# siesta-tool/SequenceDetectionQueryExecutor

Hardware: NVIDIA B200
Metric: events scanned/sec (/detection verification) (higher is better)
Workload: dtype int32

## Files before the change

### include/siesta_gpu.h

```cpp
#ifndef SIESTA_GPU_H
#define SIESTA_GPU_H

#include <stdint.h>

#ifdef __cplusplus
extern "C" {
#endif

#define SIESTA_OK 0
#define SIESTA_E_INVALID (-1)
#define SIESTA_E_CUDA (-2)
#define SIESTA_E_UNSUPPORTED (-3)
#define SIESTA_E_NOMEM (-4)
#define SIESTA_E_REFERENCE_THROWS (-5)

const char* siesta_last_error(void);

#define SIESTA_STATE_NORMAL 0
#define SIESTA_STATE_KLEENE_PLUS 1
#define SIESTA_STATE_KLEENE_STAR 2
#define SIESTA_STATE_NEGATIVE 3
#define SIESTA_STATE_OR 4

#define SIESTA_ATTR_POSITION 0
// ... 73 lines not shown
int siesta_init(int32_t device_id, siesta_ctx** out);
void siesta_shutdown(siesta_ctx* ctx);

int siesta_log_load(siesta_ctx* ctx, const int64_t* trace_off, const int32_t* act,
                    const int64_t* ts_ms, int64_t n_traces, int64_t n_events,
                    int32_t n_activities, siesta_log** out);
int siesta_log_wrap_device(siesta_ctx* ctx, const int64_t* d_trace_off, const int32_t* d_act,
                           const int64_t* d_ts_ms, int64_t n_traces, int64_t n_events,
                           int32_t n_activities, int32_t max_trace_len, siesta_log** out);
void siesta_log_set_first_trace(siesta_log* log, int64_t first_trace);
#define SIESTA_MAX_BLOCKS 16
int siesta_log_set_blocks(siesta_log* log, int32_t n_blocks, const int64_t* local_first, const int64_t* global_first);
void siesta_log_free(siesta_log* log);
int64_t siesta_log_n_traces(const siesta_log* log);
int64_t siesta_log_n_events(const siesta_log* log);

int siesta_log_filter_time(siesta_log* log, int64_t from_ms, int32_t has_from, int64_t till_ms, int32_t has_till,
                           siesta_log** out);
int siesta_log_group(siesta_log* log, const int64_t* group_off, const int64_t* group_traces, int32_t n_groups,
                     const int32_t* types, int32_t n_types, siesta_log** out, int32_t* group_ids, int32_t* n_kept);
int siesta_log_source_events(siesta_log* log, int64_t* out);

int siesta_log_append(siesta_log* log, const int64_t* trace_idx, const int64_t* batch_off, int64_t n_listed,
                      const int32_t* act, const int64_t* ts_ms, int64_t n_new_traces, int32_t n_activities,
                      siesta_log** out, double* kernel_ms);
int siesta_log_read(siesta_log* log, int64_t t0, int64_t t1, int64_t* trace_off, int32_t* act, int64_t* ts_ms);

#define SIESTA_F_RETURN_ALL 1u
#define SIESTA_F_ONLY_APPEARANCES 2u
#define SIESTA_F_MODE_HEAD 4u
// ... 199 lines not shown
```

### sequencedetectionqueryexecutor_b200/_lib.py

```python
import ctypes as C
import os

from . import _abi

_HERE = os.path.dirname(os.path.abspath(__file__))
LIB_PATH = os.environ.get("SIESTA_GPU_LIB") or os.path.join(_HERE, "libsiesta_gpu.so")
_lib = None

EXPORTS = [
    "siesta_last_error", "siesta_pattern_compile", "siesta_init", "siesta_shutdown", "siesta_log_load",
    "siesta_log_wrap_device", "siesta_log_free", "siesta_log_n_traces", "siesta_log_n_events", "siesta_detect",
    "siesta_matches_free", "siesta_evaluate_events", "siesta_evaluate_events_act8", "siesta_detect_device", "siesta_detect_device_begin", "siesta_detect_device_finish", "siesta_dev_matches_free",
    "siesta_kernel_launches", "siesta_declare_counts_size", "siesta_declare_counts", "siesta_declare_counts_device",
    "siesta_index_load", "siesta_index_build", "siesta_index_free", "siesta_index_list_len", "siesta_index_get_list",
    "siesta_intersect", "siesta_intersect_device", "siesta_device_free", "siesta_pattern_extract_pairs",
    "siesta_candidates", "siesta_candidates_device", "siesta_pair_stats", "siesta_pair_stats_device",
    "siesta_explore_accurate", "siesta_why_not_match", "siesta_almost_matches_free", "siesta_log_set_first_trace", "siesta_log_set_blocks",
    "siesta_packed_block_bytes", "siesta_dev_matches_pack",
    "siesta_exchange_create", "siesta_exchange_export", "siesta_exchange_import", "siesta_exchange_connect_local",
    "siesta_exchange_free", "siesta_exchange_required_bytes", "siesta_detect_allgather", "siesta_exchange_allreduce_i64",
    "siesta_multi_init", "siesta_multi_shutdown", "siesta_multi_n_devices", "siesta_multi_log_load", "siesta_multi_log_free",
    "siesta_multi_log_shard", "siesta_multi_detect", "siesta_multi_declare_counts", "siesta_multi_why_not_match",
    "siesta_log_filter_time", "siesta_log_group", "siesta_log_source_events",
    "siesta_log_append", "siesta_log_read", "siesta_multi_log_append",
]


class SiestaError(RuntimeError):
    def __init__(self, code, msg):
        super().__init__(f"libsiesta_gpu error {code}: {msg}")
        self.code = code


def lib():
    global _lib
    if _lib is not None:
        return _lib
    if not os.path.exists(LIB_PATH):
        raise ImportError(f"{LIB_PATH} is missing: build it with `make -C {os.path.join(_HERE, 'csrc')}` "
# ... 8 lines not shown
    L.siesta_shutdown.restype = None
    L.siesta_log_load.argtypes = [vp, vp, vp, vp, i64, i64, i32, P(vp)]
    L.siesta_log_wrap_device.argtypes = [vp, vp, vp, vp, i64, i64, i32, i32, P(vp)]
    L.siesta_packed_block_bytes.argtypes = [i64, i64, i64, i64, i32]
    L.siesta_packed_block_bytes.restype = i64
    L.siesta_dev_matches_pack.argtypes = [vp, P(_abi.DevMatches), u32, i64, vp, i64, vp]
    L.siesta_log_set_first_trace.argtypes = [vp, i64]
    L.siesta_log_set_first_trace.restype = None
    L.siesta_log_set_blocks.argtypes = [vp, i32, P(i64), P(i64)]
    L.siesta_log_free.argtypes = [vp]
    L.siesta_log_free.restype = None
    L.siesta_log_n_traces.argtypes = [vp]
    L.siesta_log_n_traces.restype = i64
    L.siesta_log_n_events.argtypes = [vp]
    L.siesta_log_n_events.restype = i64
    L.siesta_detect.argtypes = [vp, P(_abi.Nfa), vp, i64, u32, P(P(_abi.Matches))]
    L.siesta_matches_free.argtypes = [P(_abi.Matches)]
    L.siesta_matches_free.restype = None
    L.siesta_evaluate_events.argtypes = [vp, vp, vp, vp, i64, i64, i32, P(_abi.Nfa), u32, P(P(_abi.Matches))]
    L.siesta_evaluate_events_act8.argtypes = [vp, vp, vp, vp, i64, i64, i32, P(_abi.Nfa), u32, P(P(_abi.Matches))]
    L.siesta_detect_device.argtypes = [vp, P(_abi.Nfa), vp, i64, u32, vp, P(_abi.DevMatches)]
    L.siesta_detect_device_begin.argtypes = [vp, P(_abi.Nfa), vp, i64, u32, vp, P(vp)]
    L.siesta_detect_device_finish.argtypes = [vp, P(_abi.DevMatches)]
    L.siesta_dev_matches_free.argtypes = [P(_abi.DevMatches)]
    L.siesta_dev_matches_free.restype = None
    L.siesta_kernel_launches.restype = i64
    L.siesta_declare_counts_size.argtypes = [i32, i32]
    L.siesta_declare_counts_size.restype = i64
    L.siesta_declare_counts.argtypes = [vp, i32, vp, P(C.c_double)]
    L.siesta_declare_counts_device.argtypes = [vp, i32, vp, vp, P(C.c_double)]
# ... 58 lines not shown
```

### sequencedetectionqueryexecutor_b200/api.py

```python
import ctypes as C

import numpy as np

from . import _abi
from ._lib import check, lib


def _ptr(a):
    return C.c_void_p(a.ctypes.data) if a is not None else None


def _batch(trace_idx, batch_off, act, ts_ms):
    out = (np.ascontiguousarray(trace_idx, dtype=np.int64), np.ascontiguousarray(batch_off, dtype=np.int64),
           np.ascontiguousarray(act, dtype=np.int32), np.ascontiguousarray(ts_ms, dtype=np.int64))
    if len(out[1]) != len(out[0]) + 1:
        raise ValueError("batch_off must have one entry more than trace_idx")
    if len(out[2]) != len(out[3]):
        raise ValueError("act and ts_ms must have the same length")
    if out[1][-1] != len(out[2]):
        raise ValueError(f"batch_off[-1] = {int(out[1][-1])} but act / ts_ms hold {len(out[2])} events")
    return out


class Context:
# ... 60 lines not shown
            self._keep = device_tensors
            check(lib().siesta_log_wrap_device(ctx._h, C.c_void_p(d_off.data_ptr()), C.c_void_p(d_act.data_ptr()),
                                               C.c_void_p(d_ts.data_ptr()), d_off.numel() - 1, d_act.numel(),
                                               self.n_activities, int(max_trace_len), C.byref(self._h)))
        self.n_traces = lib().siesta_log_n_traces(self._h)
        self.n_events = lib().siesta_log_n_events(self._h)

    @classmethod
    def _adopt(cls, ctx, handle, n_activities):
        self = cls.__new__(cls)
        self.ctx, self._h, self.n_activities, self._keep = ctx, handle, int(n_activities), None
        self.n_traces = lib().siesta_log_n_traces(handle)
        self.n_events = lib().siesta_log_n_events(handle)
        return self

    def filter_time(self, from_ms=None, till_ms=None):
        h = C.c_void_p()
        check(lib().siesta_log_filter_time(self._h, int(from_ms or 0), 0 if from_ms is None else 1, int(till_ms or 0),
                                           0 if till_ms is None else 1, C.byref(h)))
        return EventLog._adopt(self.ctx, h, self.n_activities)

    def group(self, groups, types):
        off = np.zeros(len(groups) + 1, dtype=np.int64)
        np.cumsum([len(g) for g in groups], out=off[1:])
        flat = np.array([t for g in groups for t in g], dtype=np.int64)
        ty = np.asarray(sorted(set(types)), dtype=np.int32)
        gids = np.zeros(max(len(groups), 1), dtype=np.int32)
        h, k = C.c_void_p(), C.c_int32(0)
        check(lib().siesta_log_group(self._h, _ptr(off), _ptr(flat) if len(flat) else None, len(groups), _ptr(ty), len(ty), C.byref(h),
                                     _ptr(gids), C.byref(k)))
# ... 382 lines not shown
```

### sequencedetectionqueryexecutor_b200/csrc/append.cu

```cuda
#include <algorithm>
#include <cstring>
#include <string>
#include <vector>

#include "common.cuh"

namespace siesta {

constexpr int AP_T = 256;
constexpr int64_t AP_TILE = 8192;

__global__ void __launch_bounds__(AP_T) ap_offsets_kernel(const int64_t* __restrict__ old_off, int64_t T, int64_t T2,
                                                         const int64_t* __restrict__ tidx, const int64_t* __restrict__ boff,
                                                         int64_t k, int64_t* __restrict__ new_off, int64_t* __restrict__ P,
                                                         unsigned long long* max_len) {
    const int64_t t = (int64_t)blockIdx.x * AP_T + threadIdx.x;
    unsigned long long len = 0;
    if (t <= T2) {
        int64_t lo = 0, hi = k;
        while (lo < hi) {
            const int64_t mid = (lo + hi) >> 1;
            if (tidx[mid] < t) lo = mid + 1; else hi = mid;
        }
        const int64_t o = old_off[t < T ? t : T];
// ... 191 lines not shown
    unsigned long long h_max = 0;
    if ((e = cudaGetLastError()) == cudaSuccess) e = cudaEventRecord(ev1, stream);
    if (e == cudaSuccess) e = cudaMemcpyAsync(&h_max, d_max, 8, cudaMemcpyDeviceToHost, stream);
    if (e == cudaSuccess) e = cudaStreamSynchronize(stream);
    float ms = 0.f;
    if (e == cudaSuccess) e = cudaEventElapsedTime(&ms, ev0, ev1);
    if (e != cudaSuccess) return fail(SIESTA_E_CUDA, std::string("rebuild: ") + cudaGetErrorString(e));

    Log batch;
    batch.ctx = c;
    batch.d_act = d_bact;
    batch.n_activities = n_activities;
    batch.act_valid = true;
    if (validate_act_range(&batch, 0, NB, stream) != SIESTA_OK) return fail(SIESTA_E_CUDA, siesta_last_error());
    cudaFreeAsync(stage, stream);
    cudaEventDestroy(ev0);
    cudaEventDestroy(ev1);

    Log* L = new Log();
    L->ctx = c;
    L->d_trace_off = d_off;
    L->d_act = d_act;
    L->d_ts_ms = d_ts;
    L->n_traces = T2;
    L->n_events = E2;
    L->n_activities = n_activities;
    L->max_trace_len = (int32_t)(h_max > 0x7fffffffull ? 0x7fffffffull : h_max);
    L->true_max_len = (int64_t)h_max;
    L->owns = true;
    L->first_trace = S->first_trace;
    L->act_valid = S->act_valid && batch.act_valid;
    if (kernel_ms) *kernel_ms = ms;
    *out = reinterpret_cast<siesta_log*>(L);
    return SIESTA_OK;
}

extern "C" int siesta_log_read(siesta_log* log, int64_t t0, int64_t t1, int64_t* trace_off, int32_t* act, int64_t* ts_ms) {
    Log* L = reinterpret_cast<Log*>(log);
    if (!L || !trace_off || (!act) != (!ts_ms)) {
        set_error("siesta_log_read: null argument (act and ts_ms are both given or both NULL)");
        return SIESTA_E_INVALID;
    }
    if (t0 < 0 || t1 < t0 || t1 > L->n_traces) {
        set_error("siesta_log_read: need 0 <= t0 <= t1 <= n_traces");
        return SIESTA_E_INVALID;
    }
// ... 13 lines not shown
```

### sequencedetectionqueryexecutor_b200/csrc/capi.cu

```cuda
#include <algorithm>
#include <cstdlib>
#include <cstring>
#include <vector>

#include "common.cuh"

namespace siesta {

static thread_local std::string t_last_error;
std::atomic<long long> g_kernel_launches{0};

void set_error(const std::string& msg) { t_last_error = msg; }

}

using namespace siesta;

extern "C" const char* siesta_last_error(void) { return t_last_error.c_str(); }
extern "C" int64_t siesta_kernel_launches(void) { return (int64_t)g_kernel_launches.load(); }

extern "C" int siesta_init(int32_t device_id, siesta_ctx** out) {
    if (!out) return SIESTA_E_INVALID;
    int n_dev = 0;
    cudaError_t e = cudaGetDeviceCount(&n_dev);
// ... 85 lines not shown
}
}

extern "C" void siesta_shutdown(siesta_ctx* ctx) {
    if (!ctx) return;
    Ctx* c = reinterpret_cast<Ctx*>(ctx);
    cudaSetDevice(c->device);
    cudaDeviceSynchronize();
    for (DevBlock& b : c->dev_arena) cudaFree(b.p);
    if (c->stream) cudaStreamDestroy(c->stream);
    for (HostBlock& b : c->arena) cudaFreeHost(b.p);
    for (void* p : c->pinned_slabs) cudaFreeHost(p);
    delete c;
}

__global__ void act_range_kernel(const int32_t* act, int64_t n, int32_t n_act, int* bad) {
    int any = 0;
    for (int64_t i = (int64_t)blockIdx.x * blockDim.x + threadIdx.x; i < n; i += (int64_t)gridDim.x * blockDim.x)
        any |= (unsigned)act[i] >= (unsigned)n_act;
    if (__any_sync(0xffffffffu, any) && (threadIdx.x & 31) == 0) atomicOr(bad, 1);
}

namespace siesta {
int validate_act_range(Log* L, int64_t first_event, int64_t n_events, cudaStream_t stream) {
    if (n_events == 0) return SIESTA_OK;
    Ctx* c = L->ctx;
    int* d_bad = nullptr;
    SIESTA_CUDA_OK(cudaMallocAsync((void**)&d_bad, sizeof(int), stream));
    SIESTA_CUDA_OK(cudaMemsetAsync(d_bad, 0, sizeof(int), stream));
    const int64_t want = (n_events + 255) / 256;
    const int grid = (int)(want < (int64_t)c->sm_count * 16 ? want : (int64_t)c->sm_count * 16);
    act_range_kernel<<<grid, 256, 0, stream>>>(L->d_act + first_event, n_events, L->n_activities, d_bad);
    SIESTA_LAUNCHED();
    int bad = 1;
    SIESTA_CUDA_OK(cudaMemcpyAsync(&bad, d_bad, sizeof(int), cudaMemcpyDeviceToHost, stream));
    SIESTA_CUDA_OK(cudaStreamSynchronize(stream));
    cudaFreeAsync(d_bad, stream);
    if (bad) L->act_valid = false;
    return SIESTA_OK;
}
}

__global__ void csr_check_kernel(const int64_t* off, int64_t n_traces, int64_t n_events, int* bad) {
    int any = 0;
    for (int64_t i = (int64_t)blockIdx.x * blockDim.x + threadIdx.x; i <= n_traces; i += (int64_t)gridDim.x * blockDim.x) {
        const int64_t v = off[i];
        if (v < 0 || v > n_events) any = 1;
        if (i == 0 && v != 0) any = 1;
        if (i == n_traces && v != n_events) any = 1;
        if (i < n_traces && off[i + 1] < v) any = 1;
    }
    if (__any_sync(0xffffffffu, any) && (threadIdx.x & 31) == 0) atomicOr(bad, 1);
}

// ... 7 lines not shown
        ~Free() { cudaFreeAsync(p, s); }
    } guard{d_bad, c->stream};
    SIESTA_CUDA_OK(cudaMemsetAsync(d_bad, 0, sizeof(int), c->stream));
    const int64_t want = (L->n_traces + 1 + 255) / 256;
    const int grid = (int)(want < (int64_t)c->sm_count * 16 ? want : (int64_t)c->sm_count * 16);
    csr_check_kernel<<<grid, 256, 0, c->stream>>>(L->d_trace_off, L->n_traces, L->n_events, d_bad);
    SIESTA_LAUNCHED();
    int bad = 1;
    SIESTA_CUDA_OK(cudaMemcpyAsync(&bad, d_bad, sizeof(int), cudaMemcpyDeviceToHost, c->stream));
    SIESTA_CUDA_OK(cudaStreamSynchronize(c->stream));
    if (bad) {
        set_error("siesta_log_wrap_device: trace_off must start at 0, be non-decreasing and end at n_events");
        return SIESTA_E_INVALID;
    }
    return SIESTA_OK;
}

static int validate_act(Log* L) {
    L->act_valid = true;
    return validate_act_range(L, 0, L->n_events, L->ctx->stream);
}

static int check_csr(const int64_t* trace_off, int64_t n_traces, int64_t n_events, int32_t* max_len) {
    if (n_traces < 0 || n_events < 0 || trace_off[0] != 0 || trace_off[n_traces] != n_events) {
        set_error("CSR log: trace_off must start at 0 and end at n_events");
        return SIESTA_E_INVALID;
    }
    int64_t mx = 0;
    for (int64_t t = 0; t < n_traces; ++t) {
        const int64_t len = trace_off[t + 1] - trace_off[t];
        if (len < 0) {
            set_error("CSR log: trace_off must be non-decreasing");
            return SIESTA_E_INVALID;
        }
        mx = len > mx ? len : mx;
// ... 32 lines not shown
        delete L;
        return SIESTA_E_NOMEM;
    }
    L->d_trace_off = (const int64_t*)d_off;
    L->d_act = (const int32_t*)d_act;
    L->d_ts_ms = (const int64_t*)d_ts;
    e = cudaMemcpyAsync(d_off, trace_off, (size_t)(n_traces + 1) * 8, cudaMemcpyHostToDevice, c->stream);
    if (e == cudaSuccess && n_events) e = cudaMemcpyAsync(d_act, act, (size_t)n_events * 4, cudaMemcpyHostToDevice, c->stream);
    if (e == cudaSuccess && n_events) e = cudaMemcpyAsync(d_ts, ts_ms, (size_t)n_events * 8, cudaMemcpyHostToDevice, c->stream);
    if (e == cudaSuccess) e = cudaStreamSynchronize(c->stream);
    if (e != cudaSuccess) {
        set_error(std::string("siesta_log_load: host -> device copy: ") + cudaGetErrorString(e));
        siesta_log_free(reinterpret_cast<siesta_log*>(L));
        return SIESTA_E_CUDA;
    }
    if ((rc = validate_act(L))) {
        siesta_log_free(reinterpret_cast<siesta_log*>(L));
        return rc;
    }
    *out = reinterpret_cast<siesta_log*>(L);
    return SIESTA_OK;
}

extern "C" int siesta_log_wrap_device(siesta_ctx* ctx, const int64_t* d_trace_off, const int32_t* d_act,
                                      const int64_t* d_ts_ms, int64_t n_traces, int64_t n_events, int32_t n_activities,
                                      int32_t max_trace_len, siesta_log** out) {
    if (!ctx || !d_trace_off || !out || n_traces < 0 || n_events < 0 || n_activities < 0 || (n_events > 0 && (!d_act || !d_ts_ms))) {
        set_error("siesta_log_wrap_device: bad argument (null column with n_events > 0?)");
        return SIESTA_E_INVALID;
    }
    Log* L = new Log();
    L->ctx = reinterpret_cast<Ctx*>(ctx);
    L->d_trace_off = d_trace_off;
    L->d_act = d_act;
    L->d_ts_ms = d_ts_ms;
    L->n_traces = n_traces;
    L->n_events = n_events;
    L->n_activities = n_activities;
    L->max_trace_len = max_trace_len;
    L->owns = false;
    int rc = cudaSetDevice(L->ctx->device) == cudaSuccess ? SIESTA_OK : SIESTA_E_CUDA;
    if (rc == SIESTA_OK) rc = validate_device_csr(L);
    if (rc == SIESTA_OK) rc = validate_act(L);
    if (rc) {
        delete L;
        return rc;
    }
    *out = reinterpret_cast<siesta_log*>(L);
    return SIESTA_OK;
}

extern "C" void siesta_log_set_first_trace(siesta_log* log, int64_t first_trace) {
    if (log) reinterpret_cast<Log*>(log)->first_trace = first_trace;
}

extern "C" int siesta_log_set_blocks(siesta_log* log, int32_t n_blocks, const int64_t* local_first, const int64_t* global_first) {
    Log* L = reinterpret_cast<Log*>(log);
    if (!L || n_blocks < 0 || n_blocks > SIESTA_MAX_BLOCKS || (n_blocks > 0 && (!local_first || !global_first))) {
// ... 12 lines not shown
    }
    L->n_blocks = n_blocks;
    return SIESTA_OK;
}

extern "C" void siesta_log_free(siesta_log* log) {
    if (!log) return;
    Log* L = reinterpret_cast<Log*>(log);
    if (L->owns) {
        cudaSetDevice(L->ctx->device);
        cudaFree((void*)L->d_trace_off);
        cudaFree((void*)L->d_act);
        cudaFree((void*)L->d_ts_ms);
        if (L->d_src_event) cudaFree((void*)L->d_src_event);
    }
    delete L;
}

extern "C" int64_t siesta_log_n_traces(const siesta_log* log) { return log ? reinterpret_cast<const Log*>(log)->n_traces : 0; }
extern "C" int64_t siesta_log_n_events(const siesta_log* log) { return log ? reinterpret_cast<const Log*>(log)->n_events : 0; }

namespace {
constexpr uint64_t RESULT_MAGIC = 0x5349455354414d31ull;
constexpr size_t PIN_THRESHOLD = 256 * 1024;
constexpr size_t ARENA_KEEP_BYTES = (size_t)4 << 30;

struct ResultHeader {
    uint64_t magic;
    Ctx* ctx;
    void* base;
    uint64_t pad[5];
};
static_assert(sizeof(ResultHeader) == 64, "ResultHeader is one cache line");

void* arena_alloc(Ctx* c, size_t bytes) {
// ... 332 lines not shown
            if (!ts_mapped) ok(cudaMemcpyAsync(d_ts + e0, ts_ms + e0, (size_t)(e1 - e0) * 8, cudaMemcpyHostToDevice, s_copy));
        }
        ok(cudaEventCreateWithFlags(&copied[k], cudaEventDisableTiming));
        ok(cudaEventRecord(copied[k], s_copy));
        ok(cudaStreamWaitEvent(s_prep, copied[k], 0));
        if (e1 > e0 && e == cudaSuccess) {
            const int64_t n = e1 - e0;
            if (act8) {
                const int64_t want = (n / 4 + 256) / 256;
                const int grid = (int)std::max<int64_t>(1, std::min<int64_t>(want, (int64_t)c->sm_count * 8));
                widen_act8_kernel<<<grid, 256, 0, s_prep>>>(d_act8, d_act, e0, e1);
                SIESTA_LAUNCHED();
            }
            const int64_t want = (n + 255) / 256;
            const int grid = (int)std::max<int64_t>(1, std::min<int64_t>(want, (int64_t)c->sm_count * 16));
            act_range_kernel<<<grid, 256, 0, s_prep>>>(d_act + e0, n, n_activities, d_bad + k);
            SIESTA_LAUNCHED();
        }
        ok(cudaMemcpyAsync(h_bad + k, d_bad + k, sizeof(int), cudaMemcpyDeviceToHost, s_prep));
        ok(cudaEventCreateWithFlags(&ready[k], cudaEventDisableTiming));
        ok(cudaEventRecord(ready[k], s_prep));
    };
    struct Streamed {
        bool on = false;
        char* base = nullptr;
        siesta_matches* m = nullptr;
        cudaStream_t s = nullptr;
        std::vector<cudaEvent_t> done;
        int64_t a_tr = 0, a_occ = 0, a_ev = 0, a_err = 0, a_unsup = 0, n_emit = 0;
        bool counted = true;
        double k_ms = 0, d_ms = 0;
// ... 189 lines not shown
```

### sequencedetectionqueryexecutor_b200/csrc/common.cuh

```cuda
#pragma once
#include <cuda_runtime.h>
#include <stdint.h>

#include <atomic>
#include <mutex>
#include <string>
#include <vector>

#include "../../include/siesta_gpu.h"

namespace siesta {

void set_error(const std::string& msg);
struct Ctx;
void* dev_arena_alloc(Ctx* c, size_t bytes);
void dev_arena_free(Ctx* c, void* p);
struct DevMatchesImpl {
    void* block = nullptr;
    Ctx* owner = nullptr;
};
extern std::atomic<long long> g_kernel_launches;

#define SIESTA_CUDA_OK(expr)                                                                      \
    do {                                                                                          \
// ... 33 lines not shown
    Ctx* ctx = nullptr;
    const int64_t* d_trace_off = nullptr;
    const int32_t* d_act = nullptr;
    const int64_t* d_ts_ms = nullptr;
    const int64_t* d_src_event = nullptr;
    int64_t n_traces = 0, n_events = 0;
    int32_t n_activities = 0;
    int32_t max_trace_len = 0;
    int64_t true_max_len = -1;
    bool owns = false;
    int64_t first_trace = 0;
    int32_t n_blocks = 0;
    int64_t blk_local[SIESTA_MAX_BLOCKS + 1] = {0};
    int64_t blk_global[SIESTA_MAX_BLOCKS] = {0};
    bool act_valid = false;
};

struct DevNfa {
    int32_t n_states;
    uint32_t init_st;
    uint32_t all2;
    uint8_t kind[SIESTA_MAX_STATES];
    uint8_t n_preds[SIESTA_MAX_STATES];
    uint8_t has_vv;
    uint8_t need_vv;
    uint8_t any_kleene;
    uint8_t merge_safe;
    uint8_t cross_safe;
    uint8_t fast_class;
    int8_t kmax[SIESTA_MAX_STATES + 1];
// ... 13 lines not shown
    uint8_t le[SIESTA_MAX_STATES][SIESTA_MAX_PREDS];
    uint8_t sh[SIESTA_MAX_STATES][SIESTA_MAX_PREDS];
    uint8_t cc[SIESTA_MAX_STATES][SIESTA_MAX_PREDS];
    uint8_t markov;
    uint8_t prev[SIESTA_MAX_STATES], m_ge[SIESTA_MAX_STATES], m_le[SIESTA_MAX_STATES];
};

int nkw_build(const DevNfa& dn, uint32_t flags, NkwProgram* out);

struct DetectPending;
struct RebaseOffsets {
    int64_t trace, occ, ev;
};
int detect_device_impl(Log* log, const siesta_nfa* nfa, const int64_t* d_cand, int64_t n_cand, uint32_t flags, cudaStream_t stream,
                       RebaseOffsets base, siesta_dev_matches* out);
int validate_act_range(Log* L, int64_t first_event, int64_t n_events, cudaStream_t stream);
bool append_check_batch(const char* fn, int64_t T, const int64_t* trace_idx, const int64_t* batch_off, int64_t n_listed,
                        const int32_t* act, const int64_t* ts_ms, int64_t n_new_traces);
int assemble_matches(Ctx* c, std::vector<siesta_dev_matches>& parts, uint32_t flags, cudaStream_t stream, siesta_matches** out,
                     const std::vector<Ctx*>* part_ctx);
int detect_device_finish_impl(DetectPending* q, siesta_dev_matches* out);
void detect_pending_set_base(DetectPending* q, RebaseOffsets base);

int validate_nfa(const siesta_nfa* nfa, uint32_t flags, DevNfa* out);

constexpr int XCHG_MAX_RANKS = 16;
constexpr size_t XCHG_CTRL_BYTES = 8192;
constexpr int64_t XCHG_ERR_CAP = 4096;
enum { XST_LIMITS = 1, XST_STAGING = 2, XST_RANGE = 4, XST_ERRCAP = 8, XST_TIMEOUT = 16 };
struct XHeader {
    unsigned long long seq;
// ... 32 lines not shown
```

### sequencedetectionqueryexecutor_b200/csrc/detect.cu

```cuda
#include <algorithm>
#include <cstdio>
#include <type_traits>
#include <cstdlib>
#include <cstring>
#include <vector>

#include "detect_common.cuh"

namespace siesta {

template <int W, int R, int NF, bool SMEM_RUNS>
struct WarpSmem {
    static constexpr int NE = ROWS_OF(W);
    static constexpr size_t famvv_off = 0;
    static constexpr size_t famvv_bytes = SMEM_RUNS ? sizeof(unsigned long long) * NF * 32 : 0;
    static constexpr size_t rmask_off = famvv_off + famvv_bytes;
    static constexpr size_t rmask_bytes = SMEM_RUNS ? sizeof(typename MaskOps<W>::T) * R * 32 : 0;
    typedef typename std::conditional<W == 1, uint16_t, uint32_t>::type small_t;
    static constexpr size_t small_off = rmask_off + rmask_bytes;
    static constexpr size_t small_bytes = sizeof(small_t) * NE * 32;
    static constexpr size_t rmeta_off = (small_off + small_bytes + 15) & ~(size_t)15;
    static constexpr size_t rmeta_bytes = SMEM_RUNS ? sizeof(uint32_t) * R * 32 : 0;
    static constexpr size_t bytes_off = rmeta_off + rmeta_bytes;
    static constexpr size_t bytes_bytes = SMEM_RUNS ? (size_t)(R + 3 * NF) * 32 : 0;
// ... 912 lines not shown
    DevBuf work(log->ctx);
    const size_t nn = (size_t)std::max<int64_t>(n, 1);
    size_t w_off = 0;
    auto carve = [&w_off](size_t bytes) {
        const size_t at = w_off;
        w_off += (bytes + 255) & ~(size_t)255;
        return at;
    };
    NkwProgram prog;
    const int nkw_space = nkw_build(dn, flags, &prog);
    std::vector<uint16_t> sigs;
    for (size_t a = 0; a < lut.size(); ++a) {
        const uint16_t sg = lut[a] & 0xFFu;
        if (sg && std::find(sigs.begin(), sigs.end(), sg) == sigs.end()) sigs.push_back(sg);
    }
    const bool use_nkp = nkw_space != NKW_NONE && (!needs_ts || return_all) && log->act_valid && log->n_activities <= 255 && !sigs.empty() && sigs.size() <= 7 &&
                         (reinterpret_cast<uintptr_t>(log->d_act) & 31u) == 0 && std::getenv("SIESTA_K1_NO_NKP") == nullptr;
    const size_t reg2 = use_nkp ? (size_t)std::max<int64_t>(cap_ev, n * (int64_t)std::max(1, n_positive)) : 0;
    const bool use_long = dn.fast_class == FAST_NK && std::getenv("SIESTA_K1_NO_LONG") == nullptr;
    const int64_t cap_long = use_long ? std::min<int64_t>(log->n_events, (int64_t)1 << 21) : 0;
    const size_t long_pool = use_long ? (size_t)std::min<int64_t>(std::max<int64_t>(log->n_events * 64, (int64_t)1 << 20), (int64_t)256 << 20) : 0;
    const size_t n_blk = (nn + GT - 1) / GT;
    const size_t o_ovf2 = use_nkp ? carve(nn * 8) : 0;
    const size_t o_unsup = carve((size_t)SIESTA_MAX_UNSUPPORTED * 8);
    const size_t o_unsup2 = use_long ? carve((size_t)SIESTA_MAX_UNSUPPORTED * 8) : 0;
    const size_t o_pool = carve(long_pool);
    const size_t o_nlut = use_nkp ? carve((size_t)(log->n_activities + 1) * 16) : 0;
    const size_t o_lut = carve(lut.size() * sizeof(uint16_t)), o_nocc = carve(nn * 4), o_stage = carve(nn * 8),
                 o_stage_occ = carve(return_all ? nn * 8 : 0), o_counters = carve(32 * 8), o_err = carve(nn * 8), o_ovf = carve(nn * 8),
                 o_blk = carve(n_blk * 3 * 8), o_top = carve(((n_blk + 1023) / 1024) * 3 * 8), o_occ_nev = carve(return_all ? ((size_t)(cap_occ + cap_long) + (use_nkp ? nn : 0)) * 4 : 0), o_pos = carve(((size_t)cap_ev + reg2 + (size_t)cap_long) * 4);
    size_t o_rank = 0, o_act = 0, o_ts = 0;
    if (all_cols) {
// ... 81 lines not shown
    P.ovf_list = b_ovf.as<int64_t>();
    P.blk_sums = b_blk.as<unsigned long long>();
    P.n_blk = (int64_t)n_blk;

    P.ovf_slot = 4;
    P.tile_slot = 16;
    h_cnt = pinned_counters_get(log->ctx);
    if (!h_cnt) {
        set_error("cudaHostAlloc (counters) failed");
        return SIESTA_E_NOMEM;
    }
    std::memset(h_cnt, 0, 128);
    if (n > 0) {
        if (use_nkp) {
            DetectParams N = P;
            N.ovf_list = reinterpret_cast<int64_t*>(wb + o_ovf2);
            N.ovf_slot = 13;
            N.tile_slot = 18;
            N.fix_ev = cap_ev;
            N.fix_np = std::max(1, n_positive);
            N.fix_occ = return_all ? cap_occ + cap_long : -1;
            std::vector<uint32_t> nlut((size_t)(log->n_activities + 1) * 4, 0u);
            std::memset(N.cls_word, 0, sizeof(N.cls_word));
            for (int a = 0; a <= log->n_activities; ++a) {
                const uint16_t sg = a < log->n_activities ? (lut[a] & 0xFFu) : 0;
                int c = 0;
                if (sg) {
                    c = (int)(std::find(sigs.begin(), sigs.end(), sg) - sigs.begin()) + 1;
                    N.cls_word[c] = sg;
                }
// ... 639 lines not shown
```

### sequencedetectionqueryexecutor_b200/csrc/detect_common.cuh

```cuda
#pragma once
#include "detect_fast.cuh"

namespace siesta {

constexpr int NT = 128;
constexpr int NT_MAX = 128;
#define ROWS_OF(W) ((W) == 1 ? 24 : 64)

struct DetectParams {
    const int64_t* trace_off;
    const int32_t* act;
    const int64_t* ts_ms;
    const int64_t* cand;
    const int64_t* work;
    int64_t n_work;
    const unsigned long long* n_work_dev;
    int32_t ovf_slot;
    int32_t tile_slot;
    const uint16_t* lut;
    uint32_t relrev[3][2];
    uint16_t cls_word[8];
    int32_t cls_act[8];
    int32_t n_planes;
    int64_t n_events;
// ... 5 lines not shown
    uint32_t* d_cnt;
    int64_t* d_stage;
    int64_t* d_stage_occ;
    int32_t* s_occ_nev;
    int32_t* s_ev_pos;
    int32_t* s_ev_rank;
    int32_t* s_ev_act;
    int64_t* s_ev_ts;
    int64_t cap_occ, cap_ev;
    int64_t fix_ev;
    int32_t fix_np;
    int64_t fix_occ;
    uint32_t st_inv[SIESTA_MAX_STATES][3];
    uint8_t st_single[SIESTA_MAX_STATES];
    const uint4* nkp_lut;
    int32_t tile_batch;
    unsigned long long* counters;
    unsigned long long* blk_sums;
    int64_t n_blk;
    int64_t* err_list;
    int64_t* ovf_list;
    int64_t ovf_cap;
};

__device__ __forceinline__ long long shfl_i64(long long v, int src) {
    int lo = __shfl_sync(0xffffffffu, (int)(v & 0xffffffffll), src);
    int hi = __shfl_sync(0xffffffffu, (int)(v >> 32), src);
    return ((long long)hi << 32) | (unsigned int)lo;
}

// ... 37 lines not shown
    const int none = P.n_act;
#pragma unroll
    for (int q = 0; q < 2; ++q) {
        const long long c = e + 8 * q;
        if (c >= o1) {
            v[2 * q] = v[2 * q + 1] = make_int4(none, none, none, none);
        } else {
            asm volatile("ld.global.nc.v8.s32 {%0,%1,%2,%3,%4,%5,%6,%7}, [%8];"
                         : "=r"(v[2 * q].x), "=r"(v[2 * q].y), "=r"(v[2 * q].z), "=r"(v[2 * q].w), "=r"(v[2 * q + 1].x),
                           "=r"(v[2 * q + 1].y), "=r"(v[2 * q + 1].z), "=r"(v[2 * q + 1].w)
                         : "l"(P.act + c));
        }
    }
}

__device__ __forceinline__ uint32_t rel_push32(uint32_t pend, uint32_t relrev, int a) {
    uint32_t t;
    asm("shl.b32 %0, %1, %2;" : "=r"(t) : "r"(relrev), "r"(a));
    return __funnelshift_r(t, pend, 31);
}
__device__ __forceinline__ uint32_t rel_push64(uint32_t pend, uint32_t relrev_a, uint32_t relrev_b, int a) {
    uint32_t t;
    const uint32_t w = ((unsigned)a < 32u) ? relrev_a : (((unsigned)a < 64u) ? relrev_b : 0u);
    asm("shl.b32 %0, %1, %2;" : "=r"(t) : "r"(w), "r"(a & 31));
    return __funnelshift_r(t, pend, 31);
}

template <int NPL, bool WIDE>
__device__ __forceinline__ void scan_block(const DetectParams& P, const int4 (&v)[8], uint32_t (&pl)[3]) {
#pragma unroll
// ... 31 lines not shown
```

### sequencedetectionqueryexecutor_b200/csrc/detect_nkp.cu

```cuda
#include "detect_common.cuh"

namespace siesta {

#ifndef SIESTA_NKP_MIN_CTAS
#define SIESTA_NKP_MIN_CTAS 8
#endif
#ifndef SIESTA_NKP_PREFETCH
#define SIESTA_NKP_PREFETCH 0
#endif

constexpr int LUT_SKEW = 8;
template <int NPL, bool RAW>
__device__ __forceinline__ void scan16(const uint4* __restrict__ lut, const int4 (&v)[4], uint32_t (&pl)[3], uint32_t& racc) {
#pragma unroll
    for (int q = 3; q >= 0; --q) {
        const int a[4] = {v[q].x, v[q].y, v[q].z, v[q].w};
#pragma unroll
        for (int i = 3; i >= 0; --i) {
            const uint4 w = lut[a[i] * LUT_SKEW];
            pl[0] = pl[0] * w.x + w.y;
            if (NPL > 1) pl[1] = pl[1] * w.x + w.z;
            if (NPL > 2) pl[2] = pl[2] * w.x + w.w;
            if (!RAW) racc = racc * 2u + w.x;
        }
    }
}

__device__ __forceinline__ int select32(uint32_t x, int r) {
    int pos = 0;
#pragma unroll
    for (int w = 16; w >= 1; w >>= 1) {
        const int c = __popc((x >> pos) & ((1u << w) - 1u));
        if (r >= c) {
            r -= c;
            pos += w;
        }
    }
    return pos;
}
__device__ __forceinline__ int select64(unsigned long long x, int r) {
    const uint32_t lo = (uint32_t)x, hi = (uint32_t)(x >> 32);
    const int c = __popc(lo);
    return r >= c ? 32 + select32(hi, r - c) : select32(lo, r);
}

template <int NPL, bool RAW, bool MARKOV>
__global__ void __launch_bounds__(NT_MAX, SIESTA_NKP_MIN_CTAS) detect_nkp_kernel(const __grid_constant__ DetectParams P, const __grid_constant__ NkwProgram prog) {
    typedef typename std::conditional<RAW, unsigned long long, uint32_t>::type mask_t;
    typedef unsigned long long u64;
    typedef NkwBits<mask_t> B;
    const int lane = threadIdx.x & 31;
    extern __shared__ uint4 s_lut_all[];
    for (int i = threadIdx.x; i < (P.n_act + 1) * LUT_SKEW; i += blockDim.x) s_lut_all[i] = P.nkp_lut[i / LUT_SKEW];
    __syncthreads();
    const uint4* s_lut = s_lut_all + (lane & (LUT_SKEW - 1));
    const bool evt_pos = (P.flags & SIESTA_F_EVT_POS) != 0;
    const bool all_cols = (P.flags & SIESTA_F_NO_EVENT_COLUMNS) == 0;
    const bool return_all = (P.flags & SIESTA_F_RETURN_ALL) != 0;
    const bool first_only = (P.flags & (SIESTA_F_COUNT_MATCHES | SIESTA_F_RETURN_ALL)) == 0;

    const long long n_work = P.n_work_dev ? (long long)__ldg(P.n_work_dev) : (long long)P.n_work;
    const long long n_tiles = (n_work + 31) / 32;
    const int batch = P.tile_batch;
    long long tile = 0, next_batch = 0, next_batch2 = 0;
    if (lane == 0) {
        tile = (long long)atomicAdd(P.counters + P.tile_slot, (unsigned long long)batch);
        next_batch = (long long)atomicAdd(P.counters + P.tile_slot, (unsigned long long)batch);
    }
    tile = shfl_i64(tile, 0);
    int left = batch;
// ... 20 lines not shown
        int64_t nci;
        long long no0, no1;
        locate(nxt, nci, no0, no1);
#endif

        const long long e0 = o0 & ~7LL;
        const int lead = (int)(o0 - e0);
        const long long span = (o1 - o0) + lead;
        bool fits = span <= 64 && ((o1 + 7) & ~7LL) <= P.n_events;
        const long long o1s = fits ? o1 : e0;
        u64 valid = 0;
        if (fits && o1 > o0) valid = (span == 64 ? ~0ull : ((1ull << (int)span) - 1ull)) & ~((1ull << lead) - 1ull);
        const bool second = __any_sync(0xffffffffu, fits && span > 32);

        uint32_t q[3] = {0u, 0u, 0u}, qb[3] = {0u, 0u, 0u}, ra = 0u, rb = 0u;
        {
            int4 A[4], B[4];
            if (second) {
                load_quarter(P, e0 + 48, o1s, A);
                load_quarter(P, e0 + 32, o1s, B);
                scan16<NPL, RAW>(s_lut, A, RAW ? qb : q, rb);
                load_quarter(P, e0 + 16, o1s, A);
                scan16<NPL, RAW>(s_lut, B, RAW ? qb : q, rb);
                load_quarter(P, e0, o1s, B);
                rb += 1u;
            } else {
                load_quarter(P, e0 + 16, o1s, A);
                load_quarter(P, e0, o1s, B);
            }
            scan16<NPL, RAW>(s_lut, A, q, ra);
            scan16<NPL, RAW>(s_lut, B, q, ra);
// ... 150 lines not shown
#endif
    }
    if (lane == 31) {
        if (acc_occ) {
            atomicAdd(P.counters + 0, acc_occ);
            atomicAdd(P.counters + 6, acc_occ);
        }
        if (acc_ev) atomicAdd(P.counters + 1, acc_ev);
        if (acc_emit) atomicAdd(P.counters + 2, acc_emit);
    }
}

namespace {
template <int NPL, bool RAW, bool MARKOV>
int launch_one(const Ctx* ctx, cudaStream_t stream, DetectParams P, const NkwProgram& prog) {
    auto kern = detect_nkp_kernel<NPL, RAW, MARKOV>;
    const size_t smem = (size_t)(P.n_act + 1) * LUT_SKEW * sizeof(uint4);
    int per_sm = 0;
    SIESTA_CUDA_OK(cudaOccupancyMaxActiveBlocksPerMultiprocessor(&per_sm, kern, NT, smem));
    if (per_sm < 1) per_sm = 1;
    if (const char* env = std::getenv("SIESTA_K1_CTAS_PER_SM")) {
        const int v = std::atoi(env);
        if (v >= 1 && v < per_sm) per_sm = v;
    }
    if (const char* env = std::getenv("SIESTA_NKP_CARVEOUT")) {
        const int v = std::atoi(env);
        if (v >= 0 && v <= 100) SIESTA_CUDA_OK(cudaFuncSetAttribute(kern, cudaFuncAttributePreferredSharedMemoryCarveout, v));
    }
    const int64_t n_tiles = (P.n_work + 31) / 32;
    const int64_t ctas_needed = (n_tiles + NT / 32 - 1) / (NT / 32);
    int grid = (int)std::min<int64_t>(ctas_needed, (int64_t)ctx->sm_count * per_sm);
// ... 28 lines not shown
```

Baseline: 550.6 billion.

## Add byte-packed activity column and scan it in the NKP detection kernel

Builds a uint8 copy of the activity column during log validation when there are at most 255 activities, and the NKP detection kernel reads 8-byte chunks of it instead of int32 quads. The LUT offset is taken straight from the byte with shifts and masks. This cuts the global memory traffic of the scan to a quarter, since the kernel is bandwidth bound on activity reads. In exchange it needs extra device memory and a conversion pass at load or append time, and the old path stays reachable through an environment variable.

```diff
diff --git a/include/siesta_gpu.h b/include/siesta_gpu.h
--- a/include/siesta_gpu.h
+++ b/include/siesta_gpu.h
@@ -111,6 +111,7 @@
 void siesta_log_free(siesta_log* log);
 int64_t siesta_log_n_traces(const siesta_log* log);
 int64_t siesta_log_n_events(const siesta_log* log);
+int64_t siesta_log_act8_bytes(const siesta_log* log);
 
 int siesta_log_filter_time(siesta_log* log, int64_t from_ms, int32_t has_from, int64_t till_ms, int32_t has_till,
                            siesta_log** out);
diff --git a/sequencedetectionqueryexecutor_b200/_lib.py b/sequencedetectionqueryexecutor_b200/_lib.py
--- a/sequencedetectionqueryexecutor_b200/_lib.py
+++ b/sequencedetectionqueryexecutor_b200/_lib.py
@@ -22,7 +22,7 @@
     "siesta_multi_init", "siesta_multi_shutdown", "siesta_multi_n_devices", "siesta_multi_log_load", "siesta_multi_log_free",
     "siesta_multi_log_shard", "siesta_multi_detect", "siesta_multi_declare_counts", "siesta_multi_why_not_match",
     "siesta_log_filter_time", "siesta_log_group", "siesta_log_source_events",
-    "siesta_log_append", "siesta_log_read", "siesta_multi_log_append",
+    "siesta_log_append", "siesta_log_read", "siesta_multi_log_append", "siesta_log_act8_bytes",
 ]
 
 
@@ -61,6 +61,8 @@
     L.siesta_log_n_traces.restype = i64
     L.siesta_log_n_events.argtypes = [vp]
     L.siesta_log_n_events.restype = i64
+    L.siesta_log_act8_bytes.argtypes = [vp]
+    L.siesta_log_act8_bytes.restype = i64
     L.siesta_detect.argtypes = [vp, P(_abi.Nfa), vp, i64, u32, P(P(_abi.Matches))]
     L.siesta_matches_free.argtypes = [P(_abi.Matches)]
     L.siesta_matches_free.restype = None
diff --git a/sequencedetectionqueryexecutor_b200/api.py b/sequencedetectionqueryexecutor_b200/api.py
--- a/sequencedetectionqueryexecutor_b200/api.py
+++ b/sequencedetectionqueryexecutor_b200/api.py
@@ -98,6 +98,10 @@
         self.n_events = lib().siesta_log_n_events(handle)
         return self
 
+    @property
+    def act8_bytes(self):
+        return lib().siesta_log_act8_bytes(self._h)
+
     def filter_time(self, from_ms=None, till_ms=None):
         h = C.c_void_p()
         check(lib().siesta_log_filter_time(self._h, int(from_ms or 0), 0 if from_ms is None else 1, int(till_ms or 0),
diff --git a/sequencedetectionqueryexecutor_b200/csrc/append.cu b/sequencedetectionqueryexecutor_b200/csrc/append.cu
--- a/sequencedetectionqueryexecutor_b200/csrc/append.cu
+++ b/sequencedetectionqueryexecutor_b200/csrc/append.cu
@@ -229,8 +229,7 @@
     batch.act_valid = true;
     if (validate_act_range(&batch, 0, NB, stream) != SIESTA_OK) return fail(SIESTA_E_CUDA, siesta_last_error());
     cudaFreeAsync(stage, stream);
-    cudaEventDestroy(ev0);
-    cudaEventDestroy(ev1);
+    stage = nullptr;
 
     Log* L = new Log();
     L->ctx = c;
@@ -245,6 +244,22 @@
     L->owns = true;
     L->first_trace = S->first_trace;
     L->act_valid = S->act_valid && batch.act_valid;
+    if (L->act_valid) {
+        float ms8 = 0.f;
+        e = cudaEventRecord(ev0, stream);
+        const int rc8 = e == cudaSuccess ? validate_log_act(L, stream) : SIESTA_E_CUDA;
+        if (rc8 == SIESTA_OK && (e = cudaEventRecord(ev1, stream)) == cudaSuccess && (e = cudaEventSynchronize(ev1)) == cudaSuccess)
+            e = cudaEventElapsedTime(&ms8, ev0, ev1);
+        if (rc8 != SIESTA_OK || e != cudaSuccess) {
+            const std::string why = rc8 != SIESTA_OK ? std::string(siesta_last_error()) : std::string(cudaGetErrorString(e));
+            L->owns = false;
+            siesta_log_free(reinterpret_cast<siesta_log*>(L));
+            return fail(SIESTA_E_CUDA, "byte activity column: " + why);
+        }
+        ms += ms8;
+    }
+    cudaEventDestroy(ev0);
+    cudaEventDestroy(ev1);
     if (kernel_ms) *kernel_ms = ms;
     *out = reinterpret_cast<siesta_log*>(L);
     return SIESTA_OK;
diff --git a/sequencedetectionqueryexecutor_b200/csrc/capi.cu b/sequencedetectionqueryexecutor_b200/csrc/capi.cu
--- a/sequencedetectionqueryexecutor_b200/csrc/capi.cu
+++ b/sequencedetectionqueryexecutor_b200/csrc/capi.cu
@@ -123,15 +123,18 @@
     delete c;
 }
 
-__global__ void act_range_kernel(const int32_t* act, int64_t n, int32_t n_act, int* bad) {
+__global__ void act_range_kernel(const int32_t* act, int64_t n, int32_t n_act, int* bad, uint8_t* act8) {
     int any = 0;
-    for (int64_t i = (int64_t)blockIdx.x * blockDim.x + threadIdx.x; i < n; i += (int64_t)gridDim.x * blockDim.x)
-        any |= (unsigned)act[i] >= (unsigned)n_act;
+    for (int64_t i = (int64_t)blockIdx.x * blockDim.x + threadIdx.x; i < n; i += (int64_t)gridDim.x * blockDim.x) {
+        const int32_t a = act[i];
+        any |= (unsigned)a >= (unsigned)n_act;
+        if (act8) act8[i] = (uint8_t)a;
+    }
     if (__any_sync(0xffffffffu, any) && (threadIdx.x & 31) == 0) atomicOr(bad, 1);
 }
 
 namespace siesta {
-int validate_act_range(Log* L, int64_t first_event, int64_t n_events, cudaStream_t stream) {
+int validate_act_range(Log* L, int64_t first_event, int64_t n_events, cudaStream_t stream, uint8_t* act8) {
     if (n_events == 0) return SIESTA_OK;
     Ctx* c = L->ctx;
     int* d_bad = nullptr;
@@ -139,7 +142,7 @@
     SIESTA_CUDA_OK(cudaMemsetAsync(d_bad, 0, sizeof(int), stream));
     const int64_t want = (n_events + 255) / 256;
     const int grid = (int)(want < (int64_t)c->sm_count * 16 ? want : (int64_t)c->sm_count * 16);
-    act_range_kernel<<<grid, 256, 0, stream>>>(L->d_act + first_event, n_events, L->n_activities, d_bad);
+    act_range_kernel<<<grid, 256, 0, stream>>>(L->d_act + first_event, n_events, L->n_activities, d_bad, act8);
     SIESTA_LAUNCHED();
     int bad = 1;
     SIESTA_CUDA_OK(cudaMemcpyAsync(&bad, d_bad, sizeof(int), cudaMemcpyDeviceToHost, stream));
@@ -147,6 +150,22 @@
     cudaFreeAsync(d_bad, stream);
     if (bad) L->act_valid = false;
     return SIESTA_OK;
+}
+
+int validate_log_act(Log* L, cudaStream_t stream) {
+    L->act_valid = true;
+    uint8_t* a8 = nullptr;
+    if (L->n_activities <= 255 && L->n_events > 0 && cudaMalloc((void**)&a8, (size_t)L->n_events + 64) != cudaSuccess) {
+        cudaGetLastError();
+        a8 = nullptr;
+    }
+    const int rc = validate_act_range(L, 0, L->n_events, stream, a8);
+    if (rc || !L->act_valid) {
+        cudaFree(a8);
+        a8 = nullptr;
+    }
+    L->d_act8 = a8;
+    return rc;
 }
 }
 
@@ -184,11 +203,6 @@
         return SIESTA_E_INVALID;
     }
     return SIESTA_OK;
-}
-
-static int validate_act(Log* L) {
-    L->act_valid = true;
-    return validate_act_range(L, 0, L->n_events, L->ctx->stream);
 }
 
 static int check_csr(const int64_t* trace_off, int64_t n_traces, int64_t n_events, int32_t* max_len) {
@@ -251,7 +265,7 @@
         siesta_log_free(reinterpret_cast<siesta_log*>(L));
         return SIESTA_E_CUDA;
     }
-    if ((rc = validate_act(L))) {
+    if ((rc = validate_log_act(L, c->stream))) {
         siesta_log_free(reinterpret_cast<siesta_log*>(L));
         return rc;
     }
@@ -278,7 +292,7 @@
     L->owns = false;
     int rc = cudaSetDevice(L->ctx->device) == cudaSuccess ? SIESTA_OK : SIESTA_E_CUDA;
     if (rc == SIESTA_OK) rc = validate_device_csr(L);
-    if (rc == SIESTA_OK) rc = validate_act(L);
+    if (rc == SIESTA_OK) rc = validate_log_act(L, L->ctx->stream);
     if (rc) {
         delete L;
         return rc;
@@ -321,11 +335,19 @@
         cudaFree((void*)L->d_ts_ms);
         if (L->d_src_event) cudaFree((void*)L->d_src_event);
     }
+    if (L->d_act8) {
+        cudaSetDevice(L->ctx->device);
+        cudaFree((void*)L->d_act8);
+    }
     delete L;
 }
 
 extern "C" int64_t siesta_log_n_traces(const siesta_log* log) { return log ? reinterpret_cast<const Log*>(log)->n_traces : 0; }
 extern "C" int64_t siesta_log_n_events(const siesta_log* log) { return log ? reinterpret_cast<const Log*>(log)->n_events : 0; }
+extern "C" int64_t siesta_log_act8_bytes(const siesta_log* log) {
+    const Log* L = reinterpret_cast<const Log*>(log);
+    return L && L->d_act8 ? L->n_events + 64 : 0;
+}
 
 namespace {
 constexpr uint64_t RESULT_MAGIC = 0x5349455354414d31ull;
@@ -688,7 +710,7 @@
             }
             const int64_t want = (n + 255) / 256;
             const int grid = (int)std::max<int64_t>(1, std::min<int64_t>(want, (int64_t)c->sm_count * 16));
-            act_range_kernel<<<grid, 256, 0, s_prep>>>(d_act + e0, n, n_activities, d_bad + k);
+            act_range_kernel<<<grid, 256, 0, s_prep>>>(d_act + e0, n, n_activities, d_bad + k, nullptr);
             SIESTA_LAUNCHED();
         }
         ok(cudaMemcpyAsync(h_bad + k, d_bad + k, sizeof(int), cudaMemcpyDeviceToHost, s_prep));
diff --git a/sequencedetectionqueryexecutor_b200/csrc/common.cuh b/sequencedetectionqueryexecutor_b200/csrc/common.cuh
--- a/sequencedetectionqueryexecutor_b200/csrc/common.cuh
+++ b/sequencedetectionqueryexecutor_b200/csrc/common.cuh
@@ -71,6 +71,7 @@
     int64_t blk_local[SIESTA_MAX_BLOCKS + 1] = {0};
     int64_t blk_global[SIESTA_MAX_BLOCKS] = {0};
     bool act_valid = false;
+    const uint8_t* d_act8 = nullptr;
 };
 
 struct DevNfa {
@@ -114,7 +115,8 @@
 };
 int detect_device_impl(Log* log, const siesta_nfa* nfa, const int64_t* d_cand, int64_t n_cand, uint32_t flags, cudaStream_t stream,
                        RebaseOffsets base, siesta_dev_matches* out);
-int validate_act_range(Log* L, int64_t first_event, int64_t n_events, cudaStream_t stream);
+int validate_act_range(Log* L, int64_t first_event, int64_t n_events, cudaStream_t stream, uint8_t* act8 = nullptr);
+int validate_log_act(Log* L, cudaStream_t stream);
 bool append_check_batch(const char* fn, int64_t T, const int64_t* trace_idx, const int64_t* batch_off, int64_t n_listed,
                         const int32_t* act, const int64_t* ts_ms, int64_t n_new_traces);
 int assemble_matches(Ctx* c, std::vector<siesta_dev_matches>& parts, uint32_t flags, cudaStream_t stream, siesta_matches** out,
diff --git a/sequencedetectionqueryexecutor_b200/csrc/detect.cu b/sequencedetectionqueryexecutor_b200/csrc/detect.cu
--- a/sequencedetectionqueryexecutor_b200/csrc/detect.cu
+++ b/sequencedetectionqueryexecutor_b200/csrc/detect.cu
@@ -950,8 +950,10 @@
         const uint16_t sg = lut[a] & 0xFFu;
         if (sg && std::find(sigs.begin(), sigs.end(), sg) == sigs.end()) sigs.push_back(sg);
     }
+    const char* int32_env = std::getenv("SIESTA_NKP_INT32");
+    const uint8_t* nkp_act8 = (int32_env && std::atoi(int32_env) == 1) ? nullptr : log->d_act8;
     const bool use_nkp = nkw_space != NKW_NONE && (!needs_ts || return_all) && log->act_valid && log->n_activities <= 255 && !sigs.empty() && sigs.size() <= 7 &&
-                         (reinterpret_cast<uintptr_t>(log->d_act) & 31u) == 0 && std::getenv("SIESTA_K1_NO_NKP") == nullptr;
+                         (nkp_act8 || (reinterpret_cast<uintptr_t>(log->d_act) & 31u) == 0) && std::getenv("SIESTA_K1_NO_NKP") == nullptr;
     const size_t reg2 = use_nkp ? (size_t)std::max<int64_t>(cap_ev, n * (int64_t)std::max(1, n_positive)) : 0;
     const bool use_long = dn.fast_class == FAST_NK && std::getenv("SIESTA_K1_NO_LONG") == nullptr;
     const int64_t cap_long = use_long ? std::min<int64_t>(log->n_events, (int64_t)1 << 21) : 0;
@@ -1063,6 +1065,7 @@
     if (n > 0) {
         if (use_nkp) {
             DetectParams N = P;
+            N.act8 = nkp_act8;
             N.ovf_list = reinterpret_cast<int64_t*>(wb + o_ovf2);
             N.ovf_slot = 13;
             N.tile_slot = 18;
diff --git a/sequencedetectionqueryexecutor_b200/csrc/detect_common.cuh b/sequencedetectionqueryexecutor_b200/csrc/detect_common.cuh
--- a/sequencedetectionqueryexecutor_b200/csrc/detect_common.cuh
+++ b/sequencedetectionqueryexecutor_b200/csrc/detect_common.cuh
@@ -43,6 +43,7 @@
     uint32_t st_inv[SIESTA_MAX_STATES][3];
     uint8_t st_single[SIESTA_MAX_STATES];
     const uint4* nkp_lut;
+    const uint8_t* act8;
     int32_t tile_batch;
     unsigned long long* counters;
     unsigned long long* blk_sums;
@@ -110,6 +111,14 @@
     }
 }
 
+__device__ __forceinline__ uint2 load_chunk8(const DetectParams& P, long long c, long long o1) {
+    if (c >= o1) {
+        const uint32_t none4 = (uint32_t)P.n_act * 0x01010101u;
+        return make_uint2(none4, none4);
+    }
+    return __ldg(reinterpret_cast<const uint2*>(P.act8 + c));
+}
+
 __device__ __forceinline__ uint32_t rel_push32(uint32_t pend, uint32_t relrev, int a) {
     uint32_t t;
     asm("shl.b32 %0, %1, %2;" : "=r"(t) : "r"(relrev), "r"(a));
diff --git a/sequencedetectionqueryexecutor_b200/csrc/detect_nkp.cu b/sequencedetectionqueryexecutor_b200/csrc/detect_nkp.cu
--- a/sequencedetectionqueryexecutor_b200/csrc/detect_nkp.cu
+++ b/sequencedetectionqueryexecutor_b200/csrc/detect_nkp.cu
@@ -11,19 +11,36 @@
 
 constexpr int LUT_SKEW = 8;
 template <int NPL, bool RAW>
+__device__ __forceinline__ void scan_slot(const uint4* __restrict__ lut, uint32_t a, uint32_t (&pl)[3], uint32_t& racc) {
+    const uint4 w = lut[a * LUT_SKEW];
+    pl[0] = pl[0] * w.x + w.y;
+    if (NPL > 1) pl[1] = pl[1] * w.x + w.z;
+    if (NPL > 2) pl[2] = pl[2] * w.x + w.w;
+    if (!RAW) racc = racc * 2u + w.x;
+}
+template <int NPL, bool RAW>
 __device__ __forceinline__ void scan16(const uint4* __restrict__ lut, const int4 (&v)[4], uint32_t (&pl)[3], uint32_t& racc) {
 #pragma unroll
     for (int q = 3; q >= 0; --q) {
         const int a[4] = {v[q].x, v[q].y, v[q].z, v[q].w};
 #pragma unroll
+        for (int i = 3; i >= 0; --i) scan_slot<NPL, RAW>(lut, (uint32_t)a[i], pl, racc);
+    }
+}
+template <int NPL, bool RAW>
+__device__ __forceinline__ void scan8(const char* __restrict__ lut_b, uint32_t lane_off, uint2 v, uint32_t (&pl)[3], uint32_t& racc) {
+    const uint32_t w[2] = {v.x, v.y};
+#pragma unroll
+    for (int h = 1; h >= 0; --h)
+#pragma unroll
         for (int i = 3; i >= 0; --i) {
-            const uint4 w = lut[a[i] * LUT_SKEW];
-            pl[0] = pl[0] * w.x + w.y;
-            if (NPL > 1) pl[1] = pl[1] * w.x + w.z;
-            if (NPL > 2) pl[2] = pl[2] * w.x + w.w;
-            if (!RAW) racc = racc * 2u + w.x;
-        }
-    }
+            const uint32_t off = ((i == 0 ? w[h] << 7 : w[h] >> (8 * i - 7)) & 0x7F80u) | lane_off;
+            const uint4 e = *reinterpret_cast<const uint4*>(lut_b + off);
+            pl[0] = pl[0] * e.x + e.y;
+            if (NPL > 1) pl[1] = pl[1] * e.x + e.z;
+            if (NPL > 2) pl[2] = pl[2] * e.x + e.w;
+            if (!RAW) racc = racc * 2u + e.x;
+        }
 }
 
 __device__ __forceinline__ int select32(uint32_t x, int r) {
@@ -44,7 +61,7 @@
     return r >= c ? 32 + select32(hi, r - c) : select32(lo, r);
 }
 
-template <int NPL, bool RAW, bool MARKOV>
+template <int NPL, bool RAW, bool MARKOV, bool ACT8>
 __global__ void __launch_bounds__(NT_MAX, SIESTA_NKP_MIN_CTAS) detect_nkp_kernel(const __grid_constant__ DetectParams P, const __grid_constant__ NkwProgram prog) {
     typedef typename std::conditional<RAW, unsigned long long, uint32_t>::type mask_t;
     typedef unsigned long long u64;
@@ -54,6 +71,9 @@
     for (int i = threadIdx.x; i < (P.n_act + 1) * LUT_SKEW; i += blockDim.x) s_lut_all[i] = P.nkp_lut[i / LUT_SKEW];
     __syncthreads();
     const uint4* s_lut = s_lut_all + (lane & (LUT_SKEW - 1));
+    const char* lut_b = reinterpret_cast<const char*>(s_lut_all);
+    const uint32_t lane_off = (uint32_t)(lane & (LUT_SKEW - 1)) * (uint32_t)sizeof(uint4);
+    static_assert(LUT_SKEW * sizeof(uint4) == 128, "scan8 builds the entry offset a * 128 + lane_off");
     const bool evt_pos = (P.flags & SIESTA_F_EVT_POS) != 0;
     const bool all_cols = (P.flags & SIESTA_F_NO_EVENT_COLUMNS) == 0;
     const bool return_all = (P.flags & SIESTA_F_RETURN_ALL) != 0;
@@ -104,7 +124,23 @@
         const bool second = __any_sync(0xffffffffu, fits && span > 32);
 
         uint32_t q[3] = {0u, 0u, 0u}, qb[3] = {0u, 0u, 0u}, ra = 0u, rb = 0u;
-        {
+        if constexpr (ACT8) {
+            uint2 c8[8];
+            if (second) {
+#pragma unroll
+                for (int k = 7; k >= 4; --k) c8[k] = load_chunk8(P, e0 + 8 * k, o1s);
+            }
+#pragma unroll
+            for (int k = 3; k >= 0; --k) c8[k] = load_chunk8(P, e0 + 8 * k, o1s);
+            if (second) {
+#pragma unroll
+                for (int k = 7; k >= 4; --k) scan8<NPL, RAW>(lut_b, lane_off, c8[k], RAW ? qb : q, rb);
+                rb += 1u;
+            }
+#pragma unroll
+            for (int k = 3; k >= 0; --k) scan8<NPL, RAW>(lut_b, lane_off, c8[k], q, ra);
+            ra += 1u;
+        } else {
             int4 A[4], B[4];
             if (second) {
                 load_quarter(P, e0 + 48, o1s, A);
@@ -285,7 +321,7 @@
 namespace {
 template <int NPL, bool RAW, bool MARKOV>
 int launch_one(const Ctx* ctx, cudaStream_t stream, DetectParams P, const NkwProgram& prog) {
-    auto kern = detect_nkp_kernel<NPL, RAW, MARKOV>;
+    auto kern = P.act8 ? detect_nkp_kernel<NPL, RAW, MARKOV, true> : detect_nkp_kernel<NPL, RAW, MARKOV, false>;
     const size_t smem = (size_t)(P.n_act + 1) * LUT_SKEW * sizeof(uint4);
     int per_sm = 0;
     SIESTA_CUDA_OK(cudaOccupancyMaxActiveBlocksPerMultiprocessor(&per_sm, kern, NT, smem));
```

New measurement: 639.9 billion, median of 6. +16.2%, better.
